# CliMA/CloudMicrophysics.jl

Hardware: AMD Instinct MI355X
Metric: grid-points/sec SB2006 2M tendency sweep (higher is better)
Workload: dtype f32

## Files before the change

cloudmicrophysics.jl_amd/csrc/cmx_sb2006_column.hip:

```cpp
#include <hip/hip_runtime.h>

#include <algorithm>
#include <type_traits>

#include "cmx_launch.hpp"
#include "cmx_sb2006.hpp"

namespace cmx {

template <typename FT> struct SbColIO {
    const FT *rho, *T, *q_tot, *q_lcl, *n_lcl, *q_rai, *n_rai;
    FT *dq_lcl, *dn_lcl, *dq_rai, *dn_rai;
    const FT *inv_dz;
    FT *precip;
    int64_t n;
    int32_t n_lev;
    double inv_n_lev;
    FastDivU32 lev_div;
};

template <typename FT> struct SedFlux { FT q_rai, n_rai, q_lcl, n_lcl; };

template <typename FT, bool CLOUD, typename CV>
__device__ __forceinline__ SedFlux<FT> sed_fluxes(const CV &cv, FT r_, FT ql, FT nl, FT qr, FT nr, FT vt_n, FT vt_m) {
    SedFlux<FT> f;
    f.q_rai = (r_ * qr) * vt_m;
    f.n_rai = (r_ * nr) * vt_n;
    f.q_lcl = FT(0);
    f.n_lcl = FT(0);
    if constexpr (CLOUD) {
        FT vc_n, vc_m;
        sb2006_cloud_velocity(cv, ql, r_, r_ * nl, vc_n, vc_m);
        f.q_lcl = (r_ * ql) * vc_m;
        f.n_lcl = (r_ * nl) * vc_n;
    }
    return f;
}

template <typename FT, bool LIMITED, int VEL, bool CLOUD, typename C>
__device__ __forceinline__ SedFlux<FT> sed_fluxes_of_point(const C &c, const CloudVelConsts<FT> &cv, FT rho, FT q_lcl, FT n_lcl,
                                                          FT q_rai, FT n_rai) {
    using M = Math<FT>;
    const FT eps = M::eps();
    const FT r_ = max0(rho), ql = max0(q_lcl), nl = max0(n_lcl);
    const FT qr = max0(q_rai), nr = max0(n_rai);
    const FT rs_rho = M::rsqrt(r_);
    const FT N_rai = r_ * nr;
    const FT L_rai = r_ * M::max(qr, eps);
    const SbRainPsd<FT> psd = sb2006_rain_psd<FT, LIMITED>(c, L_rai, M::max(N_rai, eps));
    FT vt_n, vt_m;
    sb2006_rain_velocity<FT, LIMITED, VEL>(c, r_, rs_rho, psd.l2_lam, N_rai < eps, qr < eps, vt_n, vt_m);
    SedFlux<FT> f = sed_fluxes<FT, CLOUD>(cv, r_, ql, nl, qr, nr, vt_n, vt_m);
    if (any_nan(rho, q_lcl, n_lcl, q_rai, n_rai)) f.q_rai = f.n_rai = f.q_lcl = f.n_lcl = M::nan();
    return f;
}

#ifndef CMX_COL_F32_WAVES
#define CMX_COL_F32_WAVES 4
#endif
#ifndef CMX_COL_F64_WAVES
#define CMX_COL_F64_WAVES 2
#endif
template <typename FT, bool LIMITED, int VEL, bool CLOUD, int VEC, int BS, bool INTPOW = false>
__global__ __launch_bounds__(BS) __attribute__((amdgpu_waves_per_eu(sizeof(FT) == 4 ? CMX_COL_F32_WAVES : CMX_COL_F64_WAVES))) void sb2006_column_kernel(const SbConsts<FT> c, const CloudVelConsts<FT> cv, const SbColIO<FT> io,
                                                           const int64_t first, const int64_t nvec) {
    using M = Math<FT>;
    __shared__ __align__(16) FT halo[BS + 1][4];
    const int64_t tile0 = (int64_t)blockIdx.x * (BS - 1);
    const int64_t v = tile0 + threadIdx.x;
    const bool active = v < nvec;
    const int64_t nvalid = nvec - tile0 < BS ? nvec - tile0 : BS;
    const bool owner = threadIdx.x < BS - 1;
    const int64_t i0 = first + v * VEC;

    FT rho[VEC], T[VEC], q_tot[VEC], q_lcl[VEC], n_lcl[VEC], q_rai[VEC], n_rai[VEC];
    if (active) {
        load_col<FT, VEC, true>(io.rho + first, v, rho);
        load_col<FT, VEC, true>(io.T + first, v, T);
        load_col<FT, VEC, true>(io.q_tot + first, v, q_tot);
        load_col<FT, VEC, true>(io.q_lcl + first, v, q_lcl);
        load_col<FT, VEC, true>(io.n_lcl + first, v, n_lcl);
        load_col<FT, VEC, true>(io.q_rai + first, v, q_rai);
        load_col<FT, VEC, true>(io.n_rai + first, v, n_rai);
    }
    Math<FT>::prepare();
    if (nvalid < BS && threadIdx.x == BS - 1) {
        const int64_t e = first + (tile0 + nvalid) * VEC;
        SedFlux<FT> f{FT(0), FT(0), FT(0), FT(0)};
        if (e < io.n) f = sed_fluxes_of_point<FT, LIMITED, VEL, CLOUD>(front_consts<FT>(c), cv, io.rho[e], io.q_lcl[e], io.n_lcl[e], io.q_rai[e], io.n_rai[e]);
        halo[BS][0] = f.q_rai;
        halo[BS][1] = f.n_rai;
        halo[BS][2] = f.q_lcl;
        halo[BS][3] = f.n_lcl;
    }
    FT A[VEC][4], g[VEC];
    SedFlux<FT> F[VEC];
    int64_t col = 0;
    int32_t lev = 0;
    if (active) {
        if (io.n < ((int64_t)1 << 32)) {
            const uint32_t c32 = fastdiv((uint32_t)i0, io.lev_div);
            col = c32;
            lev = (int32_t)((uint32_t)i0 - c32 * (uint32_t)io.n_lev);
        } else {
            col = (int64_t)((double)i0 * io.inv_n_lev);
            int64_t k64 = i0 - col * io.n_lev;
            if (k64 < 0) { --col; k64 += io.n_lev; }
            if (k64 >= io.n_lev) { ++col; k64 -= io.n_lev; }
            lev = (int32_t)k64;
        }
        int32_t lv = lev;
        constexpr int L = (sizeof(FT) == 4 && VEC % 2 == 0 && VEL != VEL_CHEN_GEN) ? 2 : 1;
        if constexpr (L == 1) {
#pragma unroll
            for (int k = 0; k < VEC; ++k) {
                const FT r_ = max0(rho[k]), qt = max0(q_tot[k]), ql = max0(q_lcl[k]);
                const FT qr = max0(q_rai[k]), nl = max0(n_lcl[k]), nr = max0(n_rai[k]);
                const bool poisoned = any_nan(rho[k], q_tot[k], q_lcl[k], n_lcl[k], q_rai[k], n_rai[k], T[k]);
                const SbRates<FT> p = sb2006_point<FT, LIMITED, VEL, false, INTPOW>(front_consts<FT>(c), r_, T[k], qt, ql, qr, r_ * nl, r_ * nr, nl, nr);
                F[k] = sed_fluxes<FT, CLOUD>(cv, r_, ql, nl, qr, nr, p.vt_n, p.vt_m);
                g[k] = io.inv_dz[lv] * p.inv_rho;
                if (++lv == io.n_lev) lv = 0;
                A[k][0] = (p.cond + p.au_dq_lcl) + p.ac_dq_lcl;
                A[k][1] = M::fma(p.lsc_plus_au + p.ac_dN_lcl, p.inv_rho, p.na_lcl);
                A[k][2] = M::fma(-F[k].q_rai, g[k], (p.evq + p.au_dq_rai) + p.ac_dq_rai);
                A[k][3] = M::fma(-F[k].n_rai, g[k], M::fma(((p.evN + p.au_dN_rai) + p.rsc) + p.rbr, p.inv_rho, p.na_rai));
                if constexpr (CLOUD) {
                    A[k][0] = M::fma(-F[k].q_lcl, g[k], A[k][0]);
                    A[k][1] = M::fma(-F[k].n_lcl, g[k], A[k][1]);
                }
                if (poisoned) A[k][0] = A[k][1] = A[k][2] = A[k][3] = M::nan();
                if (any_nan(rho[k], q_lcl[k], n_lcl[k], q_rai[k], n_rai[k])) F[k].q_rai = F[k].n_rai = F[k].q_lcl = F[k].n_lcl = M::nan();
            }
        } else {
            using VT = std::conditional_t<L == 2, f32x2, FT>;
            using MV = Math<VT>;
#pragma unroll
            for (int k = 0; k < VEC; k += L) {
                auto val = [k](const FT (&a)[VEC]) -> VT {
                    if constexpr (L == 2) return VT{a[k], a[k + 1]};
                    else return a[k];
                };
                const VT rho_k = val(rho), T_k = val(T), qt_k = val(q_tot), ql_k = val(q_lcl), nl_k = val(n_lcl), qr_k = val(q_rai), nr_k = val(n_rai);
                const VT r_ = max0(rho_k), qt = max0(qt_k), ql = max0(ql_k);
                const VT qr = max0(qr_k), nl = max0(nl_k), nr = max0(nr_k);
                const typename MV::Mask poisoned = nan_mask(rho_k, qt_k, ql_k, nl_k, qr_k, nr_k, T_k);
                const SbRates<VT> p = sb2006_point<VT, LIMITED, VEL, false, INTPOW>(front_consts<FT, (L == 2)>(c), r_, T_k, qt, ql, qr, r_ * nl, r_ * nr, nl, nr);
                SedFlux<VT> Fk = sed_fluxes<VT, CLOUD>(cv, r_, ql, nl, qr, nr, p.vt_n, p.vt_m);
                VT gk;
                if constexpr (L == 2) {
                    const FT dz0 = io.inv_dz[lv];
                    if (++lv == io.n_lev) lv = 0;
                    const FT dz1 = io.inv_dz[lv];
                    if (++lv == io.n_lev) lv = 0;
                    gk = VT{dz0, dz1} * p.inv_rho;
                } else {
                    gk = io.inv_dz[lv] * p.inv_rho;
                    if (++lv == io.n_lev) lv = 0;
                }
                VT Ak[4];
                Ak[0] = (p.cond + p.au_dq_lcl) + p.ac_dq_lcl;
                Ak[1] = MV::fma(p.lsc_plus_au + p.ac_dN_lcl, p.inv_rho, p.na_lcl);
                Ak[2] = MV::fma(-Fk.q_rai, gk, (p.evq + p.au_dq_rai) + p.ac_dq_rai);
                Ak[3] = MV::fma(-Fk.n_rai, gk, MV::fma(((p.evN + p.au_dN_rai) + p.rsc) + p.rbr, p.inv_rho, p.na_rai));
                if constexpr (CLOUD) {
                    Ak[0] = MV::fma(-Fk.q_lcl, gk, Ak[0]);
                    Ak[1] = MV::fma(-Fk.n_lcl, gk, Ak[1]);
                }
#pragma unroll
                for (int q = 0; q < 4; ++q) Ak[q] = poisoned ? MV::nan() : Ak[q];
                const typename MV::Mask fpoison = nan_mask(rho_k, ql_k, nl_k, qr_k, nr_k);
                Fk.q_rai = fpoison ? MV::nan() : Fk.q_rai; Fk.n_rai = fpoison ? MV::nan() : Fk.n_rai;
                Fk.q_lcl = fpoison ? MV::nan() : Fk.q_lcl; Fk.n_lcl = fpoison ? MV::nan() : Fk.n_lcl;
                if constexpr (L == 2) {
#pragma unroll
                    for (int q = 0; q < 4; ++q) { A[k][q] = Ak[q].x; A[k + 1][q] = Ak[q].y; }
                    g[k] = gk.x; g[k + 1] = gk.y;
                    F[k] = SedFlux<FT>{Fk.q_rai.x, Fk.n_rai.x, Fk.q_lcl.x, Fk.n_lcl.x};
                    F[k + 1] = SedFlux<FT>{Fk.q_rai.y, Fk.n_rai.y, Fk.q_lcl.y, Fk.n_lcl.y};
                } else {
#pragma unroll
                    for (int q = 0; q < 4; ++q) A[k][q] = Ak[q];
                    g[k] = gk;
                    F[k] = Fk;
                }
            }
        }
        halo[threadIdx.x][0] = F[0].q_rai;
        halo[threadIdx.x][1] = F[0].n_rai;
        halo[threadIdx.x][2] = F[0].q_lcl;
        halo[threadIdx.x][3] = F[0].n_lcl;
    }
    __syncthreads();
    if (!active || !owner) return;
    const int up = (threadIdx.x + 1 < nvalid) ? threadIdx.x + 1 : BS;
    const SedFlux<FT> above{halo[up][0], halo[up][1], halo[up][2], halo[up][3]};
    FT o[4][VEC];
#pragma unroll
    for (int k = 0; k < VEC; ++k) {
        const SedFlux<FT> upf = (k + 1 < VEC) ? F[k + 1 < VEC ? k + 1 : 0] : above;
        const bool top = lev == io.n_lev - 1;
        o[0][k] = A[k][0];
        o[1][k] = A[k][1];
        o[2][k] = top ? A[k][2] : M::fma(upf.q_rai, g[k], A[k][2]);
        o[3][k] = top ? A[k][3] : M::fma(upf.n_rai, g[k], A[k][3]);
        if constexpr (CLOUD) {
            o[0][k] = top ? A[k][0] : M::fma(upf.q_lcl, g[k], A[k][0]);
            o[1][k] = top ? A[k][1] : M::fma(upf.n_lcl, g[k], A[k][1]);
        }
        if (lev == 0 && io.precip) io.precip[col] = F[k].q_rai;
        if (++lev == io.n_lev) { lev = 0; ++col; }
    }
    store_col<FT, VEC, true>(io.dq_lcl + first, v, o[0]);
    store_col<FT, VEC, true>(io.dn_lcl + first, v, o[1]);
    store_col<FT, VEC, true>(io.dq_rai + first, v, o[2]);
    store_col<FT, VEC, true>(io.dn_rai + first, v, o[3]);
}

#ifndef CMX_COLUMN_BS
#define CMX_COLUMN_BS 256
#endif
constexpr int kColBS = CMX_COLUMN_BS;

template <typename FT, int VEC>
static bool launch_column(bool limited, int vel, bool cloud, bool intpow, const SbConsts<FT> &c, const CloudVelConsts<FT> &cv, const SbColIO<FT> &io,
                          int64_t first, int64_t nvec, hipStream_t s) {
    if (nvec <= 0) return true;
    const dim3 grid((unsigned)((nvec + (kColBS - 1) - 1) / (kColBS - 1))), block(kColBS);
    return dispatch([&](auto L, auto K, auto C, auto I) {
        launch_grid(sb2006_column_kernel<FT, decltype(L)::value, decltype(K)::value, decltype(C)::value, VEC, kColBS, decltype(I)::value>, grid, block, 0, s, c, cv, io, first, nvec);
    }, flag(limited), one_of<VEL_SB, VEL_CHEN, VEL_CHEN_GEN>(vel), flag(cloud), flag(intpow));
}

template <typename FT, typename WR, typename TH, typename VL, typename ST>
static int32_t column_entry(const WR *wr, const TH *tps, const VL *vel, const ST *cloud_vel, uint32_t flags, int64_t n_col, int32_t n_lev,
                            const FT *inv_dz, const FT *rho, const FT *T, const FT *q_tot, const FT *q_lcl, const FT *n_lcl, const FT *q_rai,
                            const FT *n_rai, FT *dq_lcl, FT *dn_lcl, FT *dq_rai, FT *dn_rai, FT *precip, void *stream) {
    if (!wr || !tps || !vel || n_col < 0 || n_lev < 1) return CMX_ERR_BAD_ARG;
    if (flags & ~(uint32_t)(CMX_SB2006_LIMITED | CMX_VEL_SB2006 | CMX_VEL_CHEN2022)) return CMX_ERR_BAD_ARG;
    const bool sbv = flags & CMX_VEL_SB2006, chv = flags & CMX_VEL_CHEN2022;
    if (sbv == chv) return CMX_ERR_BAD_ARG;
    if (n_col > kMaxPoints / n_lev) return CMX_ERR_UNSUPPORTED;
    const int64_t n = n_col * (int64_t)n_lev;
    if (n == 0) return CMX_OK;
    if (!inv_dz || !rho || !T || !q_tot || !q_lcl || !n_lcl || !q_rai || !n_rai || !dq_lcl || !dn_lcl || !dq_rai || !dn_rai)
        return CMX_ERR_BAD_ARG;
    if ((flags & CMX_SB2006_LIMITED) && !sb_limiters_ok(*wr)) return CMX_ERR_BAD_ARG;
    if (sbv && !sb_rain_vel_ok(*vel, (flags & CMX_SB2006_LIMITED) != 0)) return CMX_ERR_BAD_ARG;
    const SbConsts<FT> c = make_sb_consts<FT>(*wr, *tps, vel, (double)Math<FT>::eps_1m());
    const bool intpow = sb_integer_exponents(*wr);
    CloudVelConsts<FT> cv{};
    if (cloud_vel) cv = make_cloud_vel_consts<FT>(wr->seifert_beheng.pdf_c, *cloud_vel);
    const SbColIO<FT> io{rho, T, q_tot, q_lcl, n_lcl, q_rai, n_rai, dq_lcl, dn_lcl, dq_rai, dn_rai, inv_dz, precip, n, n_lev, 1.0 / (double)n_lev, make_fastdiv((uint32_t)n_lev)};
    hipStream_t s = reinterpret_cast<hipStream_t>(stream);
    const bool limited = flags & CMX_SB2006_LIMITED;
    const int velk = sbv ? VEL_SB : chen_vel_kind<FT>(vel->chen2022);
    constexpr int VEC = sizeof(FT) == 8 ? 1 : Math<FT>::VEC;
    const void *ptrs[] = {rho, T, q_tot, q_lcl, n_lcl, q_rai, n_rai, dq_lcl, dn_lcl, dq_rai, dn_rai};
    const bool cloud = cloud_vel != nullptr;
    bool known = true;
    for_each_range<FT, VEC>(ptrs, n, [&](auto vec_tag, int64_t lo, int64_t count) {
        constexpr int V = decltype(vec_tag)::value;
        known &= launch_column<FT, V>(limited, velk, cloud, intpow, c, cv, io, lo, count / V, s);
    });
    if (!known) return CMX_ERR_BAD_ARG;
    return launched();
}

}

extern "C" {

int32_t cmx_sb2006_column_tendencies_sedimentation_f32(const cmx_warm_rain_2m_f32 *warm_rain, const cmx_thermo_f32 *tps, const cmx_rain_vel_f32 *vel,
                                                       const cmx_stokes_vel_f32 *cloud_vel, uint32_t flags, int64_t n_col, int32_t n_lev,
                                                       const float *inv_dz, const float *rho, const float *T, const float *q_tot,
                                                       const float *q_lcl, const float *n_lcl, const float *q_rai, const float *n_rai,
                                                       float *dq_lcl_dt, float *dn_lcl_dt, float *dq_rai_dt, float *dn_rai_dt,
                                                       float *precip_flux, void *stream) {
    return cmx::column_entry<float>(warm_rain, tps, vel, cloud_vel, flags, n_col, n_lev, inv_dz, rho, T, q_tot, q_lcl, n_lcl, q_rai, n_rai,
                                    dq_lcl_dt, dn_lcl_dt, dq_rai_dt, dn_rai_dt, precip_flux, stream);
}
int32_t cmx_sb2006_column_tendencies_sedimentation_f64(const cmx_warm_rain_2m_f64 *warm_rain, const cmx_thermo_f64 *tps, const cmx_rain_vel_f64 *vel,
                                                       const cmx_stokes_vel_f64 *cloud_vel, uint32_t flags, int64_t n_col, int32_t n_lev,
                                                       const double *inv_dz, const double *rho, const double *T, const double *q_tot,
                                                       const double *q_lcl, const double *n_lcl, const double *q_rai, const double *n_rai,
                                                       double *dq_lcl_dt, double *dn_lcl_dt, double *dq_rai_dt, double *dn_rai_dt,
                                                       double *precip_flux, void *stream) {
    return cmx::column_entry<double>(warm_rain, tps, vel, cloud_vel, flags, n_col, n_lev, inv_dz, rho, T, q_tot, q_lcl, n_lcl, q_rai, n_rai,
                                     dq_lcl_dt, dn_lcl_dt, dq_rai_dt, dn_rai_dt, precip_flux, stream);
}

}
```

Before: 119.7 billion.

## Restructure SB2006 column kernel: packed f32x2 flux state, additive NaN poison, branchless tops

Reworks the column sedimentation kernel so the per-point rates and fluxes stay in packed f32x2 form through the halo exchange and the final FMA stage, instead of unpacking into scalar arrays. NaN poisoning becomes an addition of a NaN-or-zero value rather than conditional selects. The inv_dz loads are hoisted ahead of the compute loop with 32-bit addressing. The top-level and precipitation handling is made branchless when n_lev >= VEC. Loads and stores switch to workgroup-based base-offset helpers. The aim is fewer VALU ops, registers and branches, at the cost of more complex indexing and reliance on new helpers such as load_col_wg and m_or.

Result: slower. 117.5 billion (-1.8%).

```diff
diff --git a/cloudmicrophysics.jl_amd/csrc/cmx_sb2006_column.hip b/cloudmicrophysics.jl_amd/csrc/cmx_sb2006_column.hip
--- a/cloudmicrophysics.jl_amd/csrc/cmx_sb2006_column.hip
+++ b/cloudmicrophysics.jl_amd/csrc/cmx_sb2006_column.hip
@@ -35,6 +35,14 @@
         f.n_lcl = (r_ * nl) * vc_n;
     }
     return f;
+}
+template <bool CLOUD, typename FT> __device__ __forceinline__ void poison_fluxes(SedFlux<FT> &f, FT poison) {
+    f.q_rai += poison;
+    f.n_rai += poison;
+    if constexpr (CLOUD) {
+        f.q_lcl += poison;
+        f.n_lcl += poison;
+    }
 }
 
 template <typename FT, bool LIMITED, int VEL, bool CLOUD, typename C>
@@ -51,8 +59,27 @@
     FT vt_n, vt_m;
     sb2006_rain_velocity<FT, LIMITED, VEL>(c, r_, rs_rho, psd.l2_lam, N_rai < eps, qr < eps, vt_n, vt_m);
     SedFlux<FT> f = sed_fluxes<FT, CLOUD>(cv, r_, ql, nl, qr, nr, vt_n, vt_m);
-    if (any_nan(rho, q_lcl, n_lcl, q_rai, n_rai)) f.q_rai = f.n_rai = f.q_lcl = f.n_lcl = M::nan();
+    poison_fluxes<CLOUD>(f, any_nan(rho, q_lcl, n_lcl, q_rai, n_rai) ? M::nan() : FT(0));
     return f;
+}
+
+template <typename FT> __device__ __forceinline__ void nan_poisons(FT rho, FT q_lcl, FT n_lcl, FT q_rai, FT n_rai, FT T, FT q_tot, FT &flux, FT &point) {
+    const bool flux_bad = any_nan(rho, q_lcl, n_lcl, q_rai, n_rai);
+    flux = flux_bad ? Math<FT>::nan() : FT(0);
+    point = m_or(flux_bad, any_nan(T, q_tot)) ? Math<FT>::nan() : FT(0);
+}
+__device__ __forceinline__ void nan_poisons(f32x2 rho, f32x2 q_lcl, f32x2 n_lcl, f32x2 q_rai, f32x2 n_rai, f32x2 T, f32x2 q_tot, f32x2 &flux, f32x2 &point) {
+    float f0, f1, p0, p1;
+    nan_poisons(rho.x, q_lcl.x, n_lcl.x, q_rai.x, n_rai.x, T.x, q_tot.x, f0, p0);
+    nan_poisons(rho.y, q_lcl.y, n_lcl.y, q_rai.y, n_rai.y, T.y, q_tot.y, f1, p1);
+    flux = f32x2{f0, f1};
+    point = f32x2{p0, p1};
+}
+
+template <typename FT> __device__ __forceinline__ FT half_of(FT x, int) { return x; }
+__device__ __forceinline__ float half_of(f32x2 x, int e) { return e ? x.y : x.x; }
+template <typename FT> __device__ __forceinline__ FT load_level(const FT *__restrict__ inv_dz, uint32_t lv) {
+    return *reinterpret_cast<const FT *>(reinterpret_cast<const char *>(inv_dz) + (uint32_t)(lv * (uint32_t)sizeof(FT)));
 }
 
 #ifndef CMX_COL_F32_WAVES
@@ -64,27 +91,57 @@
 template <typename FT, bool LIMITED, int VEL, bool CLOUD, int VEC, int BS, bool INTPOW = false>
 __global__ __launch_bounds__(BS) __attribute__((amdgpu_waves_per_eu(sizeof(FT) == 4 ? CMX_COL_F32_WAVES : CMX_COL_F64_WAVES))) void sb2006_column_kernel(const SbConsts<FT> c, const CloudVelConsts<FT> cv, const SbColIO<FT> io,
                                                            const int64_t first, const int64_t nvec) {
-    using M = Math<FT>;
     __shared__ __align__(16) FT halo[BS + 1][4];
+    const uint32_t lane = threadIdx.x;
     const int64_t tile0 = (int64_t)blockIdx.x * (BS - 1);
-    const int64_t v = tile0 + threadIdx.x;
+    const int64_t v = tile0 + lane;
     const bool active = v < nvec;
     const int64_t nvalid = nvec - tile0 < BS ? nvec - tile0 : BS;
-    const bool owner = threadIdx.x < BS - 1;
-    const int64_t i0 = first + v * VEC;
-
-    FT rho[VEC], T[VEC], q_tot[VEC], q_lcl[VEC], n_lcl[VEC], q_rai[VEC], n_rai[VEC];
+    const bool owner = lane < BS - 1;
+    const int64_t w0 = first + tile0 * VEC;
+    const int64_t i0 = w0 + (int64_t)lane * VEC;
+    const uint32_t n_lev = (uint32_t)io.n_lev;
+    const bool one_top = VEC == 1 || n_lev >= (uint32_t)VEC;
+
+    constexpr int L = (sizeof(FT) == 4 && VEC % 2 == 0 && VEL != VEL_CHEN_GEN) ? 2 : 1;
+    constexpr int NV = VEC / L;
+    FT rho[VEC], T[VEC], q_tot[VEC], q_lcl[VEC], n_lcl[VEC], q_rai[VEC], n_rai[VEC], inv_dz[VEC];
+    int64_t col = 0;
+    uint32_t lev = 0;
     if (active) {
-        load_col<FT, VEC, true>(io.rho + first, v, rho);
-        load_col<FT, VEC, true>(io.T + first, v, T);
-        load_col<FT, VEC, true>(io.q_tot + first, v, q_tot);
-        load_col<FT, VEC, true>(io.q_lcl + first, v, q_lcl);
-        load_col<FT, VEC, true>(io.n_lcl + first, v, n_lcl);
-        load_col<FT, VEC, true>(io.q_rai + first, v, q_rai);
-        load_col<FT, VEC, true>(io.n_rai + first, v, n_rai);
+        load_col_wg<FT, VEC, true>(io.rho + w0, lane, rho);
+        load_col_wg<FT, VEC, true>(io.T + w0, lane, T);
+        load_col_wg<FT, VEC, true>(io.q_tot + w0, lane, q_tot);
+        load_col_wg<FT, VEC, true>(io.q_lcl + w0, lane, q_lcl);
+        load_col_wg<FT, VEC, true>(io.n_lcl + w0, lane, n_lcl);
+        load_col_wg<FT, VEC, true>(io.q_rai + w0, lane, q_rai);
+        load_col_wg<FT, VEC, true>(io.n_rai + w0, lane, n_rai);
+        if (io.n < ((int64_t)1 << 32)) {
+            const uint32_t c32 = fastdiv((uint32_t)i0, io.lev_div);
+            col = c32;
+            lev = (uint32_t)i0 - c32 * n_lev;
+        } else {
+            col = (int64_t)((double)i0 * io.inv_n_lev);
+            int64_t k64 = i0 - col * io.n_lev;
+            if (k64 < 0) { --col; k64 += io.n_lev; }
+            if (k64 >= io.n_lev) { ++col; k64 -= io.n_lev; }
+            lev = (uint32_t)k64;
+        }
+        if (one_top) {
+            const uint32_t past = lev - n_lev;
+#pragma unroll
+            for (int k = 0; k < VEC; ++k) inv_dz[k] = load_level(io.inv_dz, k == 0 ? lev : (lev + k < past + k ? lev + k : past + k));
+        } else {
+            uint32_t lv = lev;
+#pragma unroll
+            for (int k = 0; k < VEC; ++k) {
+                inv_dz[k] = load_level(io.inv_dz, lv);
+                if (++lv == n_lev) lv = 0;
+            }
+        }
     }
     Math<FT>::prepare();
-    if (nvalid < BS && threadIdx.x == BS - 1) {
+    if (nvalid < BS && lane == BS - 1) {
         const int64_t e = first + (tile0 + nvalid) * VEC;
         SedFlux<FT> f{FT(0), FT(0), FT(0), FT(0)};
         if (e < io.n) f = sed_fluxes_of_point<FT, LIMITED, VEL, CLOUD>(front_consts<FT>(c), cv, io.rho[e], io.q_lcl[e], io.n_lcl[e], io.q_rai[e], io.n_rai[e]);
@@ -93,128 +150,100 @@
         halo[BS][2] = f.q_lcl;
         halo[BS][3] = f.n_lcl;
     }
-    FT A[VEC][4], g[VEC];
-    SedFlux<FT> F[VEC];
-    int64_t col = 0;
-    int32_t lev = 0;
+    using VT = std::conditional_t<L == 2, f32x2, FT>;
+    using MV = Math<VT>;
+    VT A[NV][4], g[NV];
+    SedFlux<VT> F[NV];
     if (active) {
-        if (io.n < ((int64_t)1 << 32)) {
-            const uint32_t c32 = fastdiv((uint32_t)i0, io.lev_div);
-            col = c32;
-            lev = (int32_t)((uint32_t)i0 - c32 * (uint32_t)io.n_lev);
-        } else {
-            col = (int64_t)((double)i0 * io.inv_n_lev);
-            int64_t k64 = i0 - col * io.n_lev;
-            if (k64 < 0) { --col; k64 += io.n_lev; }
-            if (k64 >= io.n_lev) { ++col; k64 -= io.n_lev; }
-            lev = (int32_t)k64;
-        }
-        int32_t lv = lev;
-        constexpr int L = (sizeof(FT) == 4 && VEC % 2 == 0 && VEL != VEL_CHEN_GEN) ? 2 : 1;
-        if constexpr (L == 1) {
-#pragma unroll
-            for (int k = 0; k < VEC; ++k) {
-                const FT r_ = max0(rho[k]), qt = max0(q_tot[k]), ql = max0(q_lcl[k]);
-                const FT qr = max0(q_rai[k]), nl = max0(n_lcl[k]), nr = max0(n_rai[k]);
-                const bool poisoned = any_nan(rho[k], q_tot[k], q_lcl[k], n_lcl[k], q_rai[k], n_rai[k], T[k]);
-                const SbRates<FT> p = sb2006_point<FT, LIMITED, VEL, false, INTPOW>(front_consts<FT>(c), r_, T[k], qt, ql, qr, r_ * nl, r_ * nr, nl, nr);
-                F[k] = sed_fluxes<FT, CLOUD>(cv, r_, ql, nl, qr, nr, p.vt_n, p.vt_m);
-                g[k] = io.inv_dz[lv] * p.inv_rho;
-                if (++lv == io.n_lev) lv = 0;
-                A[k][0] = (p.cond + p.au_dq_lcl) + p.ac_dq_lcl;
-                A[k][1] = M::fma(p.lsc_plus_au + p.ac_dN_lcl, p.inv_rho, p.na_lcl);
-                A[k][2] = M::fma(-F[k].q_rai, g[k], (p.evq + p.au_dq_rai) + p.ac_dq_rai);
-                A[k][3] = M::fma(-F[k].n_rai, g[k], M::fma(((p.evN + p.au_dN_rai) + p.rsc) + p.rbr, p.inv_rho, p.na_rai));
-                if constexpr (CLOUD) {
-                    A[k][0] = M::fma(-F[k].q_lcl, g[k], A[k][0]);
-                    A[k][1] = M::fma(-F[k].n_lcl, g[k], A[k][1]);
-                }
-                if (poisoned) A[k][0] = A[k][1] = A[k][2] = A[k][3] = M::nan();
-                if (any_nan(rho[k], q_lcl[k], n_lcl[k], q_rai[k], n_rai[k])) F[k].q_rai = F[k].n_rai = F[k].q_lcl = F[k].n_lcl = M::nan();
+#pragma unroll
+        for (int j = 0; j < NV; ++j) {
+            auto val = [j](const FT (&a)[VEC]) -> VT {
+                if constexpr (L == 2) return VT{a[2 * j], a[2 * j + 1]};
+                else return a[j];
+            };
+            const VT rho_k = val(rho), T_k = val(T), qt_k = val(q_tot), ql_k = val(q_lcl), nl_k = val(n_lcl), qr_k = val(q_rai), nr_k = val(n_rai);
+            const VT r_ = max0(rho_k), qt = max0(qt_k), ql = max0(ql_k);
+            const VT qr = max0(qr_k), nl = max0(nl_k), nr = max0(nr_k);
+            VT flux_poison, poison;
+            nan_poisons(rho_k, ql_k, nl_k, qr_k, nr_k, T_k, qt_k, flux_poison, poison);
+            SbRates<VT> p;
+            if constexpr (L == 1) p = sb2006_point<FT, LIMITED, VEL, false, INTPOW>(front_consts<FT>(c), r_, T_k, qt, ql, qr, r_ * nl, r_ * nr, nl, nr);
+            else p = sb2006_point<VT, LIMITED, VEL, false, INTPOW>(front_consts<FT, (L == 2)>(c), r_, T_k, qt, ql, qr, r_ * nl, r_ * nr, nl, nr);
+            F[j] = sed_fluxes<VT, CLOUD>(cv, r_, ql, nl, qr, nr, p.vt_n, p.vt_m);
+            g[j] = val(inv_dz) * p.inv_rho;
+            A[j][0] = (p.cond + p.au_dq_lcl) + p.ac_dq_lcl;
+            A[j][1] = MV::fma(p.lsc_plus_au + p.ac_dN_lcl, p.inv_rho, p.na_lcl);
+            A[j][2] = MV::fma(-F[j].q_rai, g[j], (p.evq + p.au_dq_rai) + p.ac_dq_rai);
+            A[j][3] = MV::fma(-F[j].n_rai, g[j], MV::fma(((p.evN + p.au_dN_rai) + p.rsc) + p.rbr, p.inv_rho, p.na_rai));
+            if constexpr (CLOUD) {
+                A[j][0] = MV::fma(-F[j].q_lcl, g[j], A[j][0]);
+                A[j][1] = MV::fma(-F[j].n_lcl, g[j], A[j][1]);
             }
-        } else {
-            using VT = std::conditional_t<L == 2, f32x2, FT>;
-            using MV = Math<VT>;
-#pragma unroll
-            for (int k = 0; k < VEC; k += L) {
-                auto val = [k](const FT (&a)[VEC]) -> VT {
-                    if constexpr (L == 2) return VT{a[k], a[k + 1]};
-                    else return a[k];
-                };
-                const VT rho_k = val(rho), T_k = val(T), qt_k = val(q_tot), ql_k = val(q_lcl), nl_k = val(n_lcl), qr_k = val(q_rai), nr_k = val(n_rai);
-                const VT r_ = max0(rho_k), qt = max0(qt_k), ql = max0(ql_k);
-                const VT qr = max0(qr_k), nl = max0(nl_k), nr = max0(nr_k);
-                const typename MV::Mask poisoned = nan_mask(rho_k, qt_k, ql_k, nl_k, qr_k, nr_k, T_k);
-                const SbRates<VT> p = sb2006_point<VT, LIMITED, VEL, false, INTPOW>(front_consts<FT, (L == 2)>(c), r_, T_k, qt, ql, qr, r_ * nl, r_ * nr, nl, nr);
-                SedFlux<VT> Fk = sed_fluxes<VT, CLOUD>(cv, r_, ql, nl, qr, nr, p.vt_n, p.vt_m);
-                VT gk;
-                if constexpr (L == 2) {
-                    const FT dz0 = io.inv_dz[lv];
-                    if (++lv == io.n_lev) lv = 0;
-                    const FT dz1 = io.inv_dz[lv];
-                    if (++lv == io.n_lev) lv = 0;
-                    gk = VT{dz0, dz1} * p.inv_rho;
-                } else {
-                    gk = io.inv_dz[lv] * p.inv_rho;
-                    if (++lv == io.n_lev) lv = 0;
-                }
-                VT Ak[4];
-                Ak[0] = (p.cond + p.au_dq_lcl) + p.ac_dq_lcl;
-                Ak[1] = MV::fma(p.lsc_plus_au + p.ac_dN_lcl, p.inv_rho, p.na_lcl);
-                Ak[2] = MV::fma(-Fk.q_rai, gk, (p.evq + p.au_dq_rai) + p.ac_dq_rai);
-                Ak[3] = MV::fma(-Fk.n_rai, gk, MV::fma(((p.evN + p.au_dN_rai) + p.rsc) + p.rbr, p.inv_rho, p.na_rai));
-                if constexpr (CLOUD) {
-                    Ak[0] = MV::fma(-Fk.q_lcl, gk, Ak[0]);
-                    Ak[1] = MV::fma(-Fk.n_lcl, gk, Ak[1]);
-                }
-#pragma unroll
-                for (int q = 0; q < 4; ++q) Ak[q] = poisoned ? MV::nan() : Ak[q];
-                const typename MV::Mask fpoison = nan_mask(rho_k, ql_k, nl_k, qr_k, nr_k);
-                Fk.q_rai = fpoison ? MV::nan() : Fk.q_rai; Fk.n_rai = fpoison ? MV::nan() : Fk.n_rai;
-                Fk.q_lcl = fpoison ? MV::nan() : Fk.q_lcl; Fk.n_lcl = fpoison ? MV::nan() : Fk.n_lcl;
-                if constexpr (L == 2) {
-#pragma unroll
-                    for (int q = 0; q < 4; ++q) { A[k][q] = Ak[q].x; A[k + 1][q] = Ak[q].y; }
-                    g[k] = gk.x; g[k + 1] = gk.y;
-                    F[k] = SedFlux<FT>{Fk.q_rai.x, Fk.n_rai.x, Fk.q_lcl.x, Fk.n_lcl.x};
-                    F[k + 1] = SedFlux<FT>{Fk.q_rai.y, Fk.n_rai.y, Fk.q_lcl.y, Fk.n_lcl.y};
-                } else {
-#pragma unroll
-                    for (int q = 0; q < 4; ++q) A[k][q] = Ak[q];
-                    g[k] = gk;
-                    F[k] = Fk;
-                }
+#pragma unroll
+            for (int q = 0; q < 4; ++q) A[j][q] += poison;
+            poison_fluxes<CLOUD>(F[j], flux_poison);
+            if constexpr (L == 1 && VEC > 1) {
+                if (j + 1 < NV) asm volatile("" : "+v"(A[j][0]), "+v"(A[j][1]), "+v"(A[j][2]), "+v"(A[j][3]), "+v"(g[j]), "+v"(rho[j + 1]), "+v"(T[j + 1]), "+v"(q_tot[j + 1]));
             }
         }
-        halo[threadIdx.x][0] = F[0].q_rai;
-        halo[threadIdx.x][1] = F[0].n_rai;
-        halo[threadIdx.x][2] = F[0].q_lcl;
-        halo[threadIdx.x][3] = F[0].n_lcl;
+        halo[lane][0] = half_of(F[0].q_rai, 0);
+        halo[lane][1] = half_of(F[0].n_rai, 0);
+        halo[lane][2] = half_of(F[0].q_lcl, 0);
+        halo[lane][3] = half_of(F[0].n_lcl, 0);
     }
     __syncthreads();
     if (!active || !owner) return;
-    const int up = (threadIdx.x + 1 < nvalid) ? threadIdx.x + 1 : BS;
-    const SedFlux<FT> above{halo[up][0], halo[up][1], halo[up][2], halo[up][3]};
+    const int up = (lane + 1 < nvalid) ? lane + 1 : BS;
+    FT in[4][VEC];
+#pragma unroll
+    for (int k = 0; k < VEC; ++k) {
+        const int j = (k + 1) / L % NV, e = (k + 1) % L;
+        in[0][k] = k + 1 < VEC ? half_of(F[j].q_lcl, e) : halo[up][2];
+        in[1][k] = k + 1 < VEC ? half_of(F[j].n_lcl, e) : halo[up][3];
+        in[2][k] = k + 1 < VEC ? half_of(F[j].q_rai, e) : halo[up][0];
+        in[3][k] = k + 1 < VEC ? half_of(F[j].n_rai, e) : halo[up][1];
+    }
+    constexpr int Q0 = CLOUD ? 0 : 2;
+    if (one_top) {
+        const uint32_t kt = n_lev - 1 - lev;
+#pragma unroll
+        for (int k = 0; k < VEC; ++k)
+#pragma unroll
+            for (int q = Q0; q < 4; ++q) in[q][k] = kt == (uint32_t)k ? FT(0) : in[q][k];
+        if (io.precip) {
+            const uint32_t k0 = lev == 0 ? 0u : kt + 1;
+            FT pf = half_of(F[0].q_rai, 0);
+#pragma unroll
+            for (int k = 1; k < VEC; ++k) pf = k0 == (uint32_t)k ? half_of(F[k / L].q_rai, k % L) : pf;
+            if (k0 < (uint32_t)VEC) io.precip[col + (lev != 0)] = pf;
+        }
+    } else {
+#pragma unroll
+        for (int k = 0; k < VEC; ++k) {
+            if (lev == n_lev - 1)
+#pragma unroll
+                for (int q = Q0; q < 4; ++q) in[q][k] = FT(0);
+            if (lev == 0 && io.precip) io.precip[col] = half_of(F[k / L].q_rai, k % L);
+            if (++lev == n_lev) { lev = 0; ++col; }
+        }
+    }
     FT o[4][VEC];
 #pragma unroll
-    for (int k = 0; k < VEC; ++k) {
-        const SedFlux<FT> upf = (k + 1 < VEC) ? F[k + 1 < VEC ? k + 1 : 0] : above;
-        const bool top = lev == io.n_lev - 1;
-        o[0][k] = A[k][0];
-        o[1][k] = A[k][1];
-        o[2][k] = top ? A[k][2] : M::fma(upf.q_rai, g[k], A[k][2]);
-        o[3][k] = top ? A[k][3] : M::fma(upf.n_rai, g[k], A[k][3]);
-        if constexpr (CLOUD) {
-            o[0][k] = top ? A[k][0] : M::fma(upf.q_lcl, g[k], A[k][0]);
-            o[1][k] = top ? A[k][1] : M::fma(upf.n_lcl, g[k], A[k][1]);
-        }
-        if (lev == 0 && io.precip) io.precip[col] = F[k].q_rai;
-        if (++lev == io.n_lev) { lev = 0; ++col; }
-    }
-    store_col<FT, VEC, true>(io.dq_lcl + first, v, o[0]);
-    store_col<FT, VEC, true>(io.dn_lcl + first, v, o[1]);
-    store_col<FT, VEC, true>(io.dq_rai + first, v, o[2]);
-    store_col<FT, VEC, true>(io.dn_rai + first, v, o[3]);
+    for (int j = 0; j < NV; ++j) {
+        VT oj[4];
+#pragma unroll
+        for (int q = 0; q < 4; ++q) {
+            if (q < Q0) oj[q] = A[j][q];
+            else if constexpr (L == 2) oj[q] = MV::fma(VT{in[q][2 * j], in[q][2 * j + 1]}, g[j], A[j][q]);
+            else oj[q] = MV::fma(in[q][j], g[j], A[j][q]);
+#pragma unroll
+            for (int e = 0; e < L; ++e) o[q][L * j + e] = half_of(oj[q], e);
+        }
+    }
+    store_col_wg<FT, VEC, true>(io.dq_lcl + w0, lane, o[0]);
+    store_col_wg<FT, VEC, true>(io.dn_lcl + w0, lane, o[1]);
+    store_col_wg<FT, VEC, true>(io.dq_rai + w0, lane, o[2]);
+    store_col_wg<FT, VEC, true>(io.dn_rai + w0, lane, o[3]);
 }
 
 #ifndef CMX_COLUMN_BS
```
